# Amandaynzhou/MMT-PSM

Hardware: AMD Instinct MI355X
Metric: imgs/sec (student+teacher step, 1000x1000, AUG_K=2) (higher is better)
Workload: dtype f32

## Files before the change

### include/mmtpsm.h

```cpp
#ifndef MMTPSM_H
#define MMTPSM_H
#include <stdint.h>
#ifdef __cplusplus
extern "C" {
#endif

#define MMT_EINVAL (-22)

int mmt_version(void);

typedef struct {
  const float* feat[4];
  float* grad_feat[4];
  int H[4];
  int W[4];
  float scale[4];
  int num_levels;
  int N;
  int C;
} mmt_pyramid;

int mmt_roi_align_forward(const mmt_pyramid* pyr , const float* rois, const int32_t* levels,
                          int K, int PH, int PW, int sampling_ratio, float* out, void* stream);
int mmt_roi_align_forward_bf16(const mmt_pyramid* pyr , const float* rois, const int32_t* levels,
// ... 103 lines not shown
  const float* res;
  const float* mask;
  const float* mul;
  float* y;
  int N, H, W, Cin, Cout, KH, KW, stride, pad, Ho, Wo;
  int relu, res_mode, out_stride, out_H, out_W;
  float mask_scale;
  const void* w_planes;
  long w_plane_stride;
  const void* x_planes;
  long x_plane_stride;
  void* y_planes;
  long y_plane_stride;
  int io_bf16;
  void* y_amax;
  const void* f16_x_amax;
  const void* f16_dy_amax;
  int y_amax_stats;
  const void* f16_guard_x;
  const void* f16_guard_dy;
  const void* w_src;
  const void* w_src_scale;
  int x_planes_layout;
  void* y_rb;
  long y_rb_stride;
  const float* y_rb_scale;
  void* y_amax_next;
  int x_planes_lag;
  int y_rb_rows;
} mmt_conv_args;

int mmt_conv_forward(const mmt_conv_args* a , void* stream);
int mmt_conv_variant(const mmt_conv_args* a );
int mmt_conv_ksplit(const mmt_conv_args* a );
int mmt_conv_wants_planes(const mmt_conv_args* a );
int mmt_set_conv_precision(int mode);
int mmt_amax(const float* x, long n, const float* rowscale, long inner, int rows, float* amax , void* stream);
int mmt_amax_stats(const float* x, long n, float* slot , void* stream);
int mmt_sum_stats(const float* a, const float* b, const float* c, const float* d, float* y, long n,
                  float* slot , void* stream);
int mmt_stats_combine(const float* const* slots , int n, float* out , void* stream);
int mmt_split_planes_f16(const float* x, void* planes, long plane_stride, long n, float scale, const float* amax ,
                         float* scale_out , float* amax_next ,
                         float* zero_slot , void* stream);
int mmt_pack_weight_f16(const float* w, void* planes, long plane_stride, int Cout, int K, float scale, const float* amax,
                        float* scale_out, void* stream);
int mmt_pack_weight_flipped_f16(const float* w, const float* scale, void* planes, long plane_stride, int Cout, int KH, int KW,
                                int Cin, const float* amax, float* scale_out, void* stream);
int mmt_conv3x3_strip_f16x2(const mmt_conv_args* a , const float* s_x , const float* s_w , void* stream);
int mmt_conv_forward_f16x2(const mmt_conv_args* a , const float* x_amax , const float* s_w , void* stream);
int mmt_get_conv_precision(void);
int mmt_stem_fused(const float* x, int N, int H, int W, const float* w_s2d, const void* w_planes, long w_plane_stride,
                   const float* s_w , const float* scale, const float* shift, const float* x_slot , float* y,
                   float* y_slot , void* stream);
int mmt_c64_conv3_fused(const float* x, int N, int H, int W, const float* w2, const void* w2_planes, long w2_plane_stride,
                        const float* s_w2 , const float* scale2, const float* shift2, const float* x_slot ,
                        const float* w3, const void* w3_planes, long w3_plane_stride, const float* s_w3 , const float* scale3,
                        const float* shift3, const float* res, float* out, float* out_slot ,
                        const float* o2_scale , int o2_scale_is_amax, float* o2_amax_next ,
                        float* out_amax_next , const float* w1, const void* w1_planes, long w1_plane_stride,
                        const float* s_w1 , const float* scale1, const float* shift1, const float* out_scale ,
                        float* o1_next, float* o1_next_slot , void* stream);
int mmt_conv_wgrad_planes_splits(const mmt_conv_args* a );
int mmt_conv_wgrad_planes(const mmt_conv_args* a , const float* dy, const void* x_planes, long x_plane_stride,
                          const void* dy_planes, long dy_plane_stride, const float* s_x, const float* s_dy, const float* rowscale,
                          float* dw, float* dbias, float* workspace, void* stream);
typedef struct {
  void* fn;
  long a[16];
} mmt_call;
int mmt_replay(const mmt_call* calls , int n, int* failed_index );
int mmt_split_planes_f16_rb(const float* x, void* planes, long plane_stride, int rows, int W, int C, const float* amax,
                            float* scale_out, void* stream);
int mmt_conv_writes_rb(const mmt_conv_args* a );
typedef struct mmt_wgrad_job {
  mmt_conv_args a;
  const float* dy; const float* rowscale; float* dw; float* dbias;
  const void* x_planes; long x_plane_stride; const void* dy_planes; long dy_plane_stride; const float* s_x; const float* s_dy;
} mmt_wgrad_job;
int mmt_conv_wgrad_group_workspace(const mmt_wgrad_job* jobs , int n, long* floats_out );
int mmt_conv_wgrad_group(const mmt_wgrad_job* jobs , int n, float* workspace, long workspace_floats, void* stream);
int mmt_sum_stats_rb(const float* a, const float* b, const float* c, const float* d, float* y, int rows, int W, int C, float* slot,
                     void* planes, long plane_stride, const float* scale, float* amax_next, void* stream);
int mmt_rb_scales_update(float* state, int n, void* stream);
int mmt_conv_forward_pg(const mmt_conv_args* a , const float* s_x , const float* s_w , int tile_rows,
                        int ksplit, void* stream);
int mmt_conv_pg_plan(const mmt_conv_args* a , int* tile_rows, int* ksplit);
int mmt_conv_pg_wanted(const mmt_conv_args* a );
typedef struct { long src_off, dst_off; int Cout, K, unit0, pad; } mmt_pack_desc;
long mmt_packed_weight_elems(int Cout, int K);
int mmt_pack_weight(const float* w, void* planes, long plane_stride, int Cout, int K, void* stream);
int mmt_pack_weight_flipped(const float* w, const float* scale, void* planes, long plane_stride, int Cout, int KH, int KW,
                            int Cin, void* stream);
int mmt_split_planes(const float* x, void* planes, long plane_stride, long n, void* stream);
typedef struct { const float* w; const float* scale; void* dst; long plane_stride; int Cout, KH, KW, Cin, unit0, pad; } mmt_flip_desc;
int mmt_pack_weights_flipped(const mmt_flip_desc* descs , const int* unit_desc , int n_units, void* stream);
int mmt_pack_weights(const float* base, void* planes, long plane_stride, const mmt_pack_desc* descs ,
                     const int* unit_desc , int n_units, void* stream);
int mmt_pack_weights_f16(const float* base, void* planes, long plane_stride, const mmt_pack_desc* descs ,
                         const int* unit_desc , int n_units, int n_descs, float* stat , void* stream);
int mmt_pack_weights_flipped_f16(const mmt_flip_desc* descs , const int* unit_desc , int n_units, int n_descs,
                                 float* stat , void* stream);

int mmt_conv_wgrad_splits(const mmt_conv_args* a );
int mmt_conv_wgrad(const mmt_conv_args* a , const float* dy,
                   const float* rowscale , float* dw, float* dbias ,
                   float* workspace , void* stream);
// ... 103 lines not shown
```

### mmt-psm_amd/csrc/conv_stem.hip

```cpp
#include "conv_shared.h"

namespace {

struct StemP {
  const float* x;
  const unsigned short* wpl; long wpl_stride;
  const float* w;
  const float* scale; const float* shift;
  float* y;
  const float* x_slot;
  const float* s_w;
  unsigned* amax_out; int amax_stats;
  int N, H, W, Hc, Wc, Hp, Wp, tiles_y, tiles_x;
};

constexpr int SPH = 19, SPW = 35, SPIX = SPH * SPW;
constexpr int SPL = 672 * 32;
constexpr int SB_OFF = 2 * SPL;
constexpr int STEM_LDS = 128 * 1024;

__device__ __forceinline__ float stem_exact(const StemP& p, int n, int oy, int ox, int co) {
  float acc = 0.f;
  for (int a = 0; a < 4; a++)
    for (int b = 0; b < 4; b++) {
      const int si = oy - 2 + a, sj = ox - 2 + b;
      if ((unsigned)si >= (unsigned)p.Hc || (unsigned)sj >= (unsigned)p.Wc) continue;
      for (int ch = 0; ch < 16; ch++) {
        const int c = ch & 3;
        if (c == 3) continue;
        const float xv = p.x[(((long)n * 3 + c) * p.H + 2 * si + (ch >> 3)) * p.W + 2 * sj + ((ch >> 2) & 1)];
        acc = fmaf(xv, p.w[((co * 4 + a) * 4 + b) * 16 + ch], acc);
      }
    }
  return acc;
}

__global__ __launch_bounds__(512) void stem_fused_kernel(const StemP p) {
  extern __shared__ __attribute__((aligned(16))) float lds[];
  char* const sm = (char*)lds;
  const int tid = threadIdx.x, lane = tid & 63;
  const int wave = __builtin_amdgcn_readfirstlane(tid >> 6);
  int bid = blockIdx.x;
  const int tx = bid % p.tiles_x; bid /= p.tiles_x;
  const int ty = bid % p.tiles_y;
  const int n = bid / p.tiles_y;
  const int py0 = ty * 7, px0 = tx * 15;
  const int oy0 = 2 * py0 - 1, ox0 = 2 * px0 - 1;
  const int sy0 = oy0 - 2, sx0 = ox0 - 2;
  const F16Guard guard = f16_guard_load(p.x_slot);
  const float sx = f16_scale_of(*p.x_slot);

  if (f16_guard_bad(guard)) {
    float amx = 0.f;
    for (int o = tid; o < 7 * 15 * 64; o += 512) {
      const int co = o & 63, q = (o >> 6) % 15, j = (o >> 6) / 15;
      const int py = py0 + j, px = px0 + q;
      if (py >= p.Hp || px >= p.Wp) continue;
      float m = 0.f;
      for (int dy = -1; dy <= 1; dy++)
        for (int dx = -1; dx <= 1; dx++) {
          const int oy = 2 * py + dy, ox = 2 * px + dx;
          if ((unsigned)oy >= (unsigned)p.Hc || (unsigned)ox >= (unsigned)p.Wc) continue;
          m = fmaxf(m, fmaxf(stem_exact(p, n, oy, ox, co) * p.scale[co] + p.shift[co], 0.f));
        }
      p.y[(((long)n * p.Hp + py) * p.Wp + px) * 64 + co] = m;
      amx = fmaxf(amx, m);
    }
    if (p.amax_out && amx > 0.f) atomicMax(p.amax_out, __builtin_bit_cast(unsigned, amx));
    return;
  }

  {
    const __amdgpu_buffer_rsrc_t rs_b = __builtin_amdgcn_make_buffer_rsrc((void*)p.wpl, 0, 0x7ffffff0, 0x00020000);
#pragma unroll
    for (int i = 0; i < 8; i++) {
      const int item = wave + 8 * i, q = item >> 5, rest = item & 31;
      __builtin_amdgcn_raw_ptr_buffer_load_lds(rs_b, (lds_ptr_t)(sm + SB_OFF + item * 1024), 16,
                                               (int)((q * p.wpl_stride + (long)rest * 512 + lane * 8) * 2), 0, 0, 0);
    }
  }
  typedef float f32x2 __attribute__((ext_vector_type(2)));
#pragma unroll
  for (int rnd = 0; rnd < 3; rnd++) {
    const int item = tid + 512 * rnd;
    if (item < 2 * SPIX) {
      const int pix = item >> 1, bh = item & 1;
      const int pr = pix / SPW, pc = pix - pr * SPW;
      const int si = sy0 + pr, sj = sx0 + pc;
      f32x2 v[3];
      const bool ok = (unsigned)si < (unsigned)p.Hc && (unsigned)sj < (unsigned)p.Wc;
#pragma unroll
      for (int c = 0; c < 3; c++)
        v[c] = ok ? *(const f32x2*)(p.x + (((long)n * 3 + c) * p.H + 2 * si + bh) * p.W + 2 * sj) : f32x2{0.f, 0.f};
      uint2 o0[2], o1[2];
      split4h(f32x4{v[0][0], v[1][0], v[2][0], 0.f}, sx, o0);
      split4h(f32x4{v[0][1], v[1][1], v[2][1], 0.f}, sx, o1);
      char* const dst = sm + pix * 32 + ((bh ^ (pix >> 3)) & 1) * 16;
      *(uint4*)dst = uint4{o0[0].x, o0[0].y, o1[0].x, o1[0].y};
      *(uint4*)(dst + SPL) = uint4{o0[1].x, o0[1].y, o1[1].x, o1[1].y};
    }
  }
  asm volatile("s_waitcnt vmcnt(0) lgkmcnt(0)" ::: "memory");
  __syncthreads();

  const int lr = lane & 31, kh2 = lane >> 5;
  const int boff = SB_OFF + lr * 32 + (((kh2 ^ (lr >> 3)) & 1) << 4);
  auto a_addr = [&](int a, int ta, int tb) {
    const int pidx = (2 * wave + a + ta) * SPW + lr + tb;
    return pidx * 32 + (((kh2 ^ (pidx >> 3)) & 1) << 4);
  };
  f32x16 acc[2][2];
#pragma unroll
  for (int a = 0; a < 2; a++)
#pragma unroll
    for (int b = 0; b < 2; b++)
#pragma unroll
      for (int r = 0; r < 16; r++) acc[a][b][r] = 0.f;
  auto fread = [&](int s, f16x8 (&fa)[2][2], f16x8 (&fb)[2][2]) {
    const int ta = s >> 2, tb = s & 3;
#pragma unroll
    for (int a = 0; a < 2; a++) {
      const int ad = a_addr(a, ta, tb);
      fa[0][a] = *(const f16x8*)(sm + ad);
      fa[1][a] = *(const f16x8*)(sm + ad + SPL);
    }
#pragma unroll
    for (int q = 0; q < 2; q++)
#pragma unroll
      for (int b = 0; b < 2; b++) fb[q][b] = *(const f16x8*)(sm + boff + ((q * 16 + s) * 2 + b) * 1024);
  };
  auto mma = [&](const f16x8 (&fa)[2][2], const f16x8 (&fb)[2][2]) {
#pragma unroll
    for (int pr = 0; pr < 3; pr++) {
      const int qa = pr == 1 ? 1 : 0, qb = pr == 0 ? 1 : 0;
#pragma unroll
      for (int a = 0; a < 2; a++)
#pragma unroll
        for (int b = 0; b < 2; b++)
          acc[a][b] = __builtin_amdgcn_mfma_f32_32x32x16_f16(fa[qa][a], fb[qb][b], acc[a][b], 0, 0, 0);
    }
  };
  {
    f16x8 faP[2][2], fbP[2][2], faQ[2][2], fbQ[2][2];
    fread(0, faP, fbP);
#pragma unroll
    for (int s = 0; s < 16; s += 2) {
      fread(s + 1, faQ, fbQ);
      mma(faP, fbP);
      if (s + 2 < 16) fread(s + 2, faP, fbP);
      mma(faQ, fbQ);
    }
  }
  __syncthreads();

  const int col_l = lane & 31, rq = lane >> 5;
  const float inv = 1.f / (sx * *p.s_w);
  float sc[2], sh[2];
#pragma unroll
  for (int b = 0; b < 2; b++) { sc[b] = p.scale[b * 32 + col_l] * inv; sh[b] = p.shift[b * 32 + col_l]; }
  f32x16 m01[2];
#pragma unroll
  for (int b = 0; b < 2; b++)
#pragma unroll
    for (int r = 0; r < 16; r++) {
      const int ox = ox0 + 8 * (r >> 2) + (r & 3) + 4 * rq;
      const bool cok = (unsigned)ox < (unsigned)p.Wc;
      float v[2];
#pragma unroll
      for (int a = 0; a < 2; a++) {
        const int oy = oy0 + 2 * wave + a;
        const float t = fmaxf(acc[a][b][r] * sc[b] + sh[b], 0.f);
        v[a] = (cok && (unsigned)oy < (unsigned)p.Hc) ? t : 0.f;
      }
      acc[0][b][r] = v[0];
      m01[b][r] = fmaxf(v[0], v[1]);
    }
  float* const xr = lds;
  float* const hv = lds + 8 * 32 * 64;
#pragma unroll
  for (int b = 0; b < 2; b++)
#pragma unroll
    for (int r = 0; r < 16; r++)
      xr[(wave * 32 + 8 * (r >> 2) + (r & 3) + 4 * rq) * 64 + b * 32 + col_l] = acc[0][b][r];
  __syncthreads();
  if (wave < 7) {
#pragma unroll
    for (int b = 0; b < 2; b++)
#pragma unroll
      for (int r = 0; r < 16; r++) {
        const int col = 8 * (r >> 2) + (r & 3) + 4 * rq;
        hv[(wave * 32 + col) * 64 + b * 32 + col_l] = fmaxf(m01[b][r], xr[((wave + 1) * 32 + col) * 64 + b * 32 + col_l]);
      }
  }
  __syncthreads();
  float amx = 0.f, asum = 0.f, acnt = 0.f;
  for (int o = tid; o < 7 * 15 * 16; o += 512) {
    const int c4 = o & 15, q = (o >> 4) % 15, j = (o >> 4) / 15;
    const int py = py0 + j, px = px0 + q;
    if (py >= p.Hp || px >= p.Wp) continue;
    const f32x4* const row = (const f32x4*)(hv + (j * 32 + 2 * q) * 64) + c4;
    const f32x4 t0 = row[0], t1 = row[16], t2 = row[32];
    f32x4 m;
#pragma unroll
    for (int e = 0; e < 4; e++) {
      m[e] = fmaxf(fmaxf(t0[e], t1[e]), t2[e]);
      amx = fmaxf(amx, m[e]);
      asum += m[e];
    }
    acnt += 4.f;
    *(f32x4*)(p.y + (((long)n * p.Hp + py) * p.Wp + px) * 64 + c4 * 4) = m;
  }
  if (p.amax_out) {
    __syncthreads();
    float* const red = lds;
    const bool stats = p.amax_stats && (blockIdx.x & 63) == 0;
#pragma unroll
    for (int o = 32; o > 0; o >>= 1) amx = fmaxf(amx, __shfl_xor(amx, o, 64));
    if (stats) {
#pragma unroll
      for (int o = 32; o > 0; o >>= 1) { asum += __shfl_xor(asum, o, 64); acnt += __shfl_xor(acnt, o, 64); }
    }
    if (lane == 0) { red[wave] = amx; red[16 + wave] = asum; red[32 + wave] = acnt; }
    __syncthreads();
    if (tid == 0) {
      float m = red[0], sm_ = red[16], cn = red[32];
      for (int i = 1; i < 8; i++) { m = fmaxf(m, red[i]); sm_ += red[16 + i]; cn += red[32 + i]; }
      const unsigned bits = __builtin_bit_cast(unsigned, m);
      if (m > 0.f && bits > __hip_atomic_load(p.amax_out, __ATOMIC_RELAXED, __HIP_MEMORY_SCOPE_AGENT)) atomicMax(p.amax_out, bits);
      if (stats && cn > 0.f) {
        const int k = (blockIdx.x >> 6) & 15;
        atomicAdd((float*)p.amax_out + 1 + k, sm_);
        atomicAdd((float*)p.amax_out + 17 + k, cn);
      }
    }
  }
}


struct C64Tail {
  const unsigned short* w3pl; long w3pl_stride;
  const float* w3;
  const float* scale; const float* shift;
  const float* res;
  float* out;
  const float* s_w3;
  const float* s_o2; int s_o2_amax;
  unsigned* o2_amax_next;
  unsigned* amax_out;
  unsigned* out_amax_next;
  const unsigned short* w1pl; long w1pl_stride; const float* w1; const float* scale1; const float* shift1; const float* s_w1;
  const float* s_out; float* o1n; unsigned* amax_o1n;
};
constexpr int C64_PW = 18, C64_PIX = 180, C64_SLAB = 192 * 32, C64_PL = 4 * C64_SLAB, C64_BOFF = 2 * C64_PL;
constexpr int C64_RED = 32768;
constexpr int C64_W1B = 32768;

__device__ __forceinline__ void c64_dma16(const void* g, void* l) {
#if defined(__HIP_DEVICE_COMPILE__)
  const unsigned la = __builtin_amdgcn_readfirstlane((unsigned)(unsigned long)(__attribute__((address_space(3))) char*)l);
  asm volatile("s_mov_b32 m0, %1\n\ts_nop 0\n\tglobal_load_lds_dwordx4 %0, off" ::"v"(g), "s"(la) : "m0", "memory");
#endif
}

__device__ __forceinline__ void c64_tail_exact(const ConvP& p, const C64Tail& t, const float* lds, const int img, const int oy0, const int ox0,
                                               const int wave, const int lane, float& amx, float& asum, float& acnt) {
  const float* const o2 = lds + wave * 2048;
  for (int j = 0; j < 4; j++) {
    const int c = lane + 64 * j;
    const float* const wr = t.w3 + c * 64;
    const float sc = t.scale ? t.scale[c] : 1.f, sh = t.shift ? t.shift[c] : 0.f;
    for (int i = 0; i < 32; i++) {
      const int oy = oy0 + 2 * wave + (i >> 4), ox = ox0 + (i & 15);
      if (oy >= p.Ho || ox >= p.Wo) continue;
      float acc = 0.f;
      for (int k = 0; k < 64; k++) acc = fmaf(o2[i * 64 + k], wr[k], acc);
      const long o = ((long)(img * p.Ho + oy) * p.Wo + ox) * 256 + c;
      float v = acc * sc + sh;
      if (t.res) v += t.res[o];
      v = fmaxf(v, 0.f);
      t.out[o] = v;
      amx = fmaxf(amx, v); asum += v; acnt += 1.f;
    }
  }
}

__device__ __forceinline__ float c64_o2_exact(const ConvP& p, float* lds, const int img, const int oy0, const int ox0, const int wave,
                                              const int lane) {
// ... 497 lines not shown
}

template <int FUSE>
static int launch_c64_form(const ConvP& p, const C64Tail& t, hipStream_t s) {
  constexpr int LDS = C64_BOFF + 2 * 16384;
  static bool done = false;
  if (!done) {
    const hipError_t e = hipFuncSetAttribute((const void*)conv3x3_c64_kernel<FUSE>, hipFuncAttributeMaxDynamicSharedMemorySize, LDS);
    if (e != hipSuccess) return (int)e;
    done = true;
  }
  const int tiles = p.N * ((p.Ho + 7) >> 3) * ((p.Wo + 15) >> 4);
  hipLaunchKernelGGL(conv3x3_c64_kernel<FUSE>, dim3(tiles), dim3(256), LDS, s, p, t);
  MMT_LAUNCH_CHECK();
  return 0;
}

int launch_c64(const ConvP& p, hipStream_t s) { return launch_c64_form<0>(p, C64Tail{}, s); }
}

extern "C" int mmt_c64_conv3_fused(const float* x, int N, int H, int W, const float* w2, const void* w2_planes, long w2_plane_stride,
                                   const float* s_w2, const float* scale2, const float* shift2, const float* x_slot, const float* w3,
                                   const void* w3_planes, long w3_plane_stride, const float* s_w3, const float* scale3,
                                   const float* shift3, const float* res, float* out, float* out_slot, const float* o2_scale,
                                   int o2_scale_is_amax, float* o2_amax_next, float* out_amax_next, const float* w1,
                                   const void* w1_planes, long w1_plane_stride, const float* s_w1, const float* scale1,
                                   const float* shift1, const float* out_scale, float* o1_next, float* o1_next_slot, void* stream) {
  if (!x || !w2 || !w2_planes || !s_w2 || !x_slot || !w3 || !w3_planes || !s_w3 || !res || !out || !o2_scale || N <= 0 || H <= 0 || W <= 0 ||
      (((size_t)w2_planes | (size_t)w3_planes | (size_t)x) & 15) || ((w2_plane_stride | w3_plane_stride) & 7) ||
      (((size_t)res | (size_t)out) & 3) || precision() != 3)
    return MMT_EINVAL;
  if (w1_planes && (!w1 || !s_w1 || !out_scale || !o1_next || ((size_t)w1_planes & 15) || (w1_plane_stride & 7) || ((size_t)o1_next & 3) ||
                    (const void*)res == (const void*)out))
    return MMT_EINVAL;
  if ((long)N * H * W * 1024 >= (1L << 31)) return MMT_EINVAL;
  ConvP p = {};
  p.x = x; p.w = w2; p.scale = scale2; p.shift = shift2;
  p.N = N; p.H = p.Ho = H; p.W = p.Wo = W; p.Cin = p.Cout = 64; p.KH = p.KW = 3; p.stride = 1; p.pad = 1;
  p.relu = 1; p.out_stride = 1; p.M = N * H * W; p.K = 576; p.cin32 = p.cin4 = 1;
  p.wpl = (const unsigned short*)w2_planes; p.wpl_stride = w2_plane_stride;
  p.f16_sx = x_slot; p.f16_ax = 1; p.f16_sw = s_w2; p.guard_x = x_slot;
  C64Tail t = {};
  t.w3pl = (const unsigned short*)w3_planes; t.w3pl_stride = w3_plane_stride; t.w3 = w3; t.scale = scale3; t.shift = shift3;
  t.res = res; t.out = out; t.s_w3 = s_w3; t.s_o2 = o2_scale; t.s_o2_amax = o2_scale_is_amax ? 1 : 0;
  t.o2_amax_next = (unsigned*)o2_amax_next; t.amax_out = (unsigned*)out_slot; t.out_amax_next = (unsigned*)out_amax_next;
  if (!w1_planes) return launch_c64_form<1>(p, t, (hipStream_t)stream);
  t.w1pl = (const unsigned short*)w1_planes; t.w1pl_stride = w1_plane_stride; t.w1 = w1; t.scale1 = scale1; t.shift1 = shift1;
  t.s_w1 = s_w1; t.s_out = out_scale; t.o1n = o1_next; t.amax_o1n = (unsigned*)o1_next_slot;
  return launch_c64_form<2>(p, t, (hipStream_t)stream);
}

extern "C" int mmt_stem_fused(const float* x, int N, int H, int W, const float* w_s2d, const void* w_planes, long w_plane_stride,
                              const float* s_w, const float* scale, const float* shift, const float* x_slot, float* y, float* y_slot,
                              void* stream) {
  if (!x || !w_s2d || !w_planes || !s_w || !scale || !shift || !x_slot || !y || N <= 0 || H < 8 || W < 8 || (H & 3) || (W & 3) ||
      ((size_t)w_planes & 15) || (w_plane_stride & 7) || ((size_t)x & 7) || ((size_t)y & 15) || precision() != 3)
    return MMT_EINVAL;
  if ((long)N * 3 * H * W >= (1L << 31)) return MMT_EINVAL;
  StemP p;
  p.x = x; p.wpl = (const unsigned short*)w_planes; p.wpl_stride = w_plane_stride; p.w = w_s2d;
  p.scale = scale; p.shift = shift; p.y = y; p.x_slot = x_slot; p.s_w = s_w;
  p.amax_out = (unsigned*)y_slot; p.amax_stats = y_slot ? 1 : 0;
  p.N = N; p.H = H; p.W = W; p.Hc = H / 2; p.Wc = W / 2; p.Hp = H / 4; p.Wp = W / 4;
  p.tiles_y = mmt_cdiv(p.Hp, 7); p.tiles_x = mmt_cdiv(p.Wp, 15);
  static bool done = false;
  if (!done) {
    const hipError_t e = hipFuncSetAttribute((const void*)stem_fused_kernel, hipFuncAttributeMaxDynamicSharedMemorySize, STEM_LDS);
    if (e != hipSuccess) return (int)e;
    done = true;
  }
  hipLaunchKernelGGL(stem_fused_kernel, dim3(N * p.tiles_y * p.tiles_x), dim3(512), STEM_LDS, (hipStream_t)stream, p);
  MMT_LAUNCH_CHECK();
  return 0;
}
```

### mmt-psm_amd/maskrcnn_benchmark/_hip.py

```python
import ctypes
import weakref
import os
import threading as _threading

import torch

_HERE = os.path.dirname(os.path.abspath(__file__))
LIB_PATH = os.path.join(os.path.dirname(_HERE), "libmmtpsm.so")

c_void_p, c_int, c_float, c_double, c_int64 = ctypes.c_void_p, ctypes.c_int, ctypes.c_float, ctypes.c_double, ctypes.c_int64


class Pyramid(ctypes.Structure):
    _fields_ = [("feat", c_void_p * 4), ("grad_feat", c_void_p * 4), ("H", c_int * 4), ("W", c_int * 4),
                ("scale", c_float * 4), ("num_levels", c_int), ("N", c_int), ("C", c_int)]


class RoiMaps(ctypes.Structure):
    _fields_ = [("feat", c_void_p * 4), ("grad_feat", c_void_p * 4), ("H", c_int * 4), ("W", c_int * 4), ("C", c_int * 4),
                ("c_off", c_int * 4), ("scale", c_float * 4), ("num_maps", c_int), ("N", c_int), ("out_C", c_int)]


class ConvArgs(ctypes.Structure):
    _fields_ = [("x", c_void_p), ("w", c_void_p), ("scale", c_void_p), ("shift", c_void_p), ("res", c_void_p),
# ... 86 lines not shown
                       c_void_p, c_void_p],
    "mmt_split_planes": [c_void_p, c_void_p, ctypes.c_long, ctypes.c_long, c_void_p],
    "mmt_conv_wants_planes": [ctypes.POINTER(ConvArgs)],
    "mmt_pack_weights": [c_void_p, c_void_p, ctypes.c_long, c_void_p, c_void_p, c_int, c_void_p],
    "mmt_pack_weights_flipped": [c_void_p, c_void_p, c_int, c_void_p],
    "mmt_pack_weights_f16": [c_void_p, c_void_p, ctypes.c_long, c_void_p, c_void_p, c_int, c_int, c_void_p, c_void_p],
    "mmt_pack_weights_flipped_f16": [c_void_p, c_void_p, c_int, c_int, c_void_p, c_void_p],
    "mmt_pack_weight_flipped": [c_void_p, c_void_p, c_void_p, ctypes.c_long, c_int, c_int, c_int, c_int, c_void_p],
    "mmt_conv_wgrad_splits": [ctypes.POINTER(ConvArgs)],
    "mmt_conv_wgrad": [ctypes.POINTER(ConvArgs), c_void_p, c_void_p, c_void_p, c_void_p, c_void_p, c_void_p],
    "mmt_colsum": [c_void_p, c_int, c_int, c_void_p, c_void_p],
    "mmt_weight_flip_transpose": [c_void_p, c_void_p, c_void_p, c_int, c_int, c_int, c_int, c_void_p],
    "mmt_maxpool3x3s2": [c_void_p, c_void_p, c_int, c_int, c_int, c_int, c_int, c_int, c_void_p],
    "mmt_amax": [c_void_p, ctypes.c_long, c_void_p, ctypes.c_long, c_int, c_void_p, c_void_p],
    "mmt_amax_stats": [c_void_p, ctypes.c_long, c_void_p, c_void_p],
    "mmt_det_postprocess": [c_void_p, c_void_p, c_void_p, c_void_p, c_int, c_int, c_float, c_float, c_int, c_void_p,
                            c_void_p, c_void_p, c_void_p, c_void_p, c_void_p],
    "mmt_position_embedding": [c_void_p, c_int, c_int, c_int, c_void_p, c_void_p, c_void_p],
    "mmt_sample_fg_bg_wide": [c_void_p, c_int, c_void_p, c_void_p, c_int, c_int, c_int, c_int, c_void_p, c_void_p, c_void_p, c_void_p,
                              c_void_p],
    "mmt_rpn_loss": [c_void_p, c_void_p, c_void_p, c_void_p, c_void_p, c_void_p, ctypes.c_long, c_float, c_void_p, c_void_p, c_void_p,
                     c_void_p, c_void_p],
    "mmt_box_loss": [c_void_p, c_void_p, c_void_p, c_void_p, c_int, c_int, c_void_p, c_void_p, c_void_p, c_void_p],
    "mmt_box_loss_rows": [c_void_p, c_void_p, c_void_p, c_void_p, c_int, c_int, c_void_p, c_void_p, c_void_p, c_void_p, c_void_p],
    "mmt_relation_attention_fwd": [c_void_p, c_void_p, c_void_p, c_void_p, c_void_p, c_int, c_int, c_int, c_int, c_int, c_int, c_float,
                                   c_void_p, c_void_p, c_void_p],
    "mmt_relation_attention_bwd": [c_void_p, c_void_p, c_void_p, c_void_p, c_void_p, c_void_p, c_int, c_int, c_int, c_int, c_int, c_float,
                                   c_void_p, c_void_p, c_void_p, c_void_p, c_void_p, c_void_p],
    "mmt_ciam_fwd": [c_void_p, c_void_p, c_int, c_int, c_int, c_int, c_void_p, c_void_p, c_void_p, c_void_p, c_void_p],
    "mmt_ciam_bwd": [c_void_p, c_void_p, c_int, c_int, c_int, c_int, c_void_p, c_void_p, c_void_p, c_void_p, c_void_p, c_void_p,
                     c_void_p, c_void_p, c_void_p],
    "mmt_stats_combine": [c_void_p, c_int, c_void_p, c_void_p],
    "mmt_sum_stats": [c_void_p, c_void_p, c_void_p, c_void_p, c_void_p, ctypes.c_long, c_void_p, c_void_p],
    "mmt_split_planes_f16": [c_void_p, c_void_p, ctypes.c_long, ctypes.c_long, c_float, c_void_p, c_void_p, c_void_p, c_void_p, c_void_p],
    "mmt_split_planes_f16_rb": [c_void_p, c_void_p, ctypes.c_long, c_int, c_int, c_int, c_void_p, c_void_p, c_void_p],
    "mmt_replay": [c_void_p, c_int, c_void_p],
    "mmt_conv_writes_rb": [ctypes.POINTER(ConvArgs)],
    "mmt_conv_wgrad_group_workspace": [c_void_p, c_int, ctypes.POINTER(ctypes.c_long)],
    "mmt_conv_wgrad_group": [c_void_p, c_int, c_void_p, ctypes.c_long, c_void_p],
    "mmt_sum_stats_rb": [c_void_p, c_void_p, c_void_p, c_void_p, c_void_p, c_int, c_int, c_int, c_void_p, c_void_p, ctypes.c_long, c_void_p,
                         c_void_p, c_void_p],
    "mmt_rb_scales_update": [c_void_p, c_int, c_void_p],
    "mmt_conv_wgrad_planes_splits": [ctypes.POINTER(ConvArgs)],
    "mmt_conv_wgrad_planes": [ctypes.POINTER(ConvArgs), c_void_p, c_void_p, ctypes.c_long, c_void_p, ctypes.c_long, c_void_p, c_void_p,
                              c_void_p, c_void_p, c_void_p, c_void_p, c_void_p],
    "mmt_pack_weight_f16": [c_void_p, c_void_p, ctypes.c_long, c_int, c_int, c_float, c_void_p, c_void_p, c_void_p],
    "mmt_pack_weight_flipped_f16": [c_void_p, c_void_p, c_void_p, ctypes.c_long, c_int, c_int, c_int, c_int, c_void_p, c_void_p, c_void_p],
    "mmt_conv3x3_strip_f16x2": [ctypes.POINTER(ConvArgs), c_void_p, c_void_p, c_void_p],
    "mmt_conv_forward_f16x2": [ctypes.POINTER(ConvArgs), c_void_p, c_void_p, c_void_p],
    "mmt_conv_forward_pg": [ctypes.POINTER(ConvArgs), c_void_p, c_void_p, c_int, c_int, c_void_p],
    "mmt_conv_pg_plan": [ctypes.POINTER(ConvArgs), c_void_p, c_void_p],
    "mmt_conv_pg_wanted": [ctypes.POINTER(ConvArgs)],
    "mmt_stem_fused": [c_void_p, c_int, c_int, c_int, c_void_p, c_void_p, ctypes.c_long, c_void_p, c_void_p, c_void_p, c_void_p, c_void_p,
                       c_void_p, c_void_p],
    "mmt_c64_conv3_fused": [c_void_p, c_int, c_int, c_int, c_void_p, c_void_p, ctypes.c_long, c_void_p, c_void_p, c_void_p, c_void_p, c_void_p,
                            c_void_p, ctypes.c_long, c_void_p, c_void_p, c_void_p, c_void_p, c_void_p, c_void_p, c_void_p, c_int, c_void_p,
                            c_void_p, c_void_p, c_void_p, ctypes.c_long, c_void_p, c_void_p, c_void_p, c_void_p, c_void_p, c_void_p,
                            c_void_p],
    "mmt_maxpool3x3s2_bf16": [c_void_p, c_void_p, c_int, c_int, c_int, c_int, c_int, c_int, c_void_p],
    "mmt_gconv3x3_forward": [c_void_p, c_void_p, c_void_p, c_void_p, c_void_p, c_int, c_int, c_int, c_int, c_int, c_int, c_int, c_void_p],
    "mmt_gconv3x3_dgrad": [c_void_p, c_void_p, c_void_p, c_void_p, c_void_p, c_void_p, c_int, c_int, c_int, c_int, c_int, c_int, c_void_p],
    "mmt_gconv3x3_wgrad": [c_void_p, c_void_p, c_void_p, c_void_p, c_int, c_int, c_int, c_int, c_int, c_int, c_void_p],
    "mmt_maxpool3x3s2_backward": [c_void_p, c_void_p, c_void_p, c_int, c_int, c_int, c_int, c_void_p],
    "mmt_stem_wgrad": [c_void_p, c_void_p, c_void_p, c_void_p, c_int, c_int, c_int, c_void_p],
    "mmt_mask_bce": [c_void_p, c_void_p, c_void_p, c_int, c_int, c_int, c_float, c_void_p, c_void_p, c_void_p],
    "mmt_mgd_level_forward": [c_void_p, ctypes.POINTER(MgdTeachers), c_void_p, c_int, c_int, c_int, c_int, c_void_p, c_void_p],
    "mmt_mgd_level_backward": [c_void_p, ctypes.POINTER(MgdTeachers), c_void_p, c_int, c_int, c_int, c_int, c_void_p, c_void_p, c_void_p],
    "mmt_mgd_views_forward": [ctypes.POINTER(MgdStudents), ctypes.POINTER(MgdTeachers), c_void_p, c_int, c_int, c_int, c_int, c_void_p,
                              c_void_p],
    "mmt_mgd_views_backward": [ctypes.POINTER(MgdStudents), ctypes.POINTER(MgdTeachers), c_void_p, c_int, c_int, c_int, c_int, c_void_p,
                               c_void_p, c_void_p],
    "mmt_mask_pool": [c_void_p, c_int, c_int, c_int, c_int, c_int, c_void_p, c_void_p],
    "mmt_psm_rows": [c_void_p, c_int, c_void_p, c_int, c_int, c_void_p, c_float, c_int, c_int, c_void_p, c_void_p, c_void_p],
    "mmt_psm_variance": [c_void_p, c_int, c_int, c_int, c_int, c_void_p, c_void_p],
    "mmt_ema_update": [c_void_p, c_void_p, c_int64, c_double, c_void_p],
    "mmt_sgd_momentum": [c_void_p, c_void_p, c_void_p, c_int64, c_float, c_float, c_float, c_int, c_void_p],
    "mmt_grad_guard": [c_void_p, c_int64, c_void_p, c_void_p, c_float, c_void_p],
    "mmt_sgd_momentum_guarded": [c_void_p, c_void_p, c_void_p, c_int64, c_float, c_float, c_float, c_int, c_void_p, c_void_p],
    "mmt_paste_masks": [c_void_p, c_void_p, c_void_p, c_void_p, c_int, c_int, c_int, c_int, c_int, c_float, c_void_p, c_void_p],
    "mmt_paste_mask_stack": [c_void_p, c_void_p, c_int, c_int, c_int, c_int, c_float, c_void_p, c_void_p],
    "mmt_polygon_targets": [c_void_p, c_void_p, c_void_p, c_void_p, c_int, c_int, c_void_p, c_void_p, c_void_p],
    "mmt_mask_pack": [c_void_p, c_int, c_int, c_int, c_void_p, c_void_p, c_void_p],
    "mmt_paste_mask_words": [c_void_p, c_void_p, c_int, c_int, c_int, c_int, c_float, c_void_p, c_void_p, c_void_p],
    "mmt_mask_expand": [c_void_p, c_void_p, c_int, c_int, c_int, c_void_p, c_void_p, c_void_p],
    "mmt_mask_transition_counts": [c_void_p, c_int, c_int, c_int, c_void_p, c_void_p],
    "mmt_mask_transition_positions": [c_void_p, c_int, c_int, c_int, c_void_p, c_void_p, c_void_p],
    "mmt_mask_pair_intersections": [c_void_p, c_void_p, c_int, c_void_p, c_void_p, c_int, c_int, c_int, c_void_p, c_void_p],
    "mmt_set_deterministic": [c_int],
    "mmt_get_deterministic": [],
    "mmt_roi_align_backward_ordered": [ctypes.POINTER(Pyramid), c_void_p, c_void_p, c_int, c_int, c_int, c_int, c_void_p, c_int, c_void_p],
    "mmt_colsum_ordered": [c_void_p, c_int, c_int, c_void_p, c_void_p, c_void_p],
    "mmt_mask_bce_ordered": [c_void_p, c_void_p, c_void_p, c_int, c_int, c_int, c_float, c_void_p, c_void_p, c_void_p, c_void_p],
    "mmt_mgd_level_forward_ordered": [c_void_p, ctypes.POINTER(MgdTeachers), c_void_p, c_int, c_int, c_int, c_int, c_void_p, c_void_p, c_void_p],
    "mmt_mgd_views_forward_ordered": [ctypes.POINTER(MgdStudents), ctypes.POINTER(MgdTeachers), c_void_p, c_int, c_int, c_int, c_int, c_void_p,
                                      c_void_p, c_void_p],
    "mmt_box_loss_ordered": [c_void_p, c_void_p, c_void_p, c_void_p, c_int, c_int, c_void_p, c_void_p, c_void_p, c_void_p, c_void_p, c_void_p],
    "mmt_ciam_bwd_ordered": [c_void_p, c_void_p, c_int, c_int, c_int, c_int, c_void_p, c_void_p, c_void_p, c_void_p, c_void_p, c_void_p,
                             c_void_p, c_void_p, c_void_p, c_void_p],
}

_lib = None
PROFILE = None
PROFILE_ALL = False
_BF16_STORAGE = os.environ.get("MMT_BF16_STORAGE", "0") != "0"


F16X2_DEFAULT = os.environ.get("MMT_F16X2", "1") != "0"
# ... 1486 lines not shown
        a.y_amax, a.y_amax_stats = amax_slot.ptr, 1
    if mul is not None:
        mul = nhwc(mul)
        a.mul = mul.data_ptr()
    ebytes = _epilogue_bytes(y, res, res_mode, mask, mul) if PROFILE is not None else None
    if kind != K_LIB:
        if fast_ok and not io:
            _plan_record(x, w, f16_src, stride, pad, relu, res, res_mode, mask, a, kind, Cout, Ho, Wo)
        if amax_slot is None or mul is not None:
            rb_site = None
        return _conv_f16(a, kind, x, src, y, amax_slot, rb_site, 0, 0, None, ebytes)
    var = lib().mmt_conv_variant(ctypes.byref(a)) if ebytes is not None else 0
    rec = ebytes is not None and (var in (1, 4) or PROFILE_ALL)
    pre = None
    if auto_split:
        p0 = _ev() if rec else None
        split_planes(x, x_planes)
        if rec:
            pre = (p0, _ev())
    e0 = _ev() if rec else None
    if planes_owner is not None:
        planes_owner.ensure_bf16()
    _check(lib().mmt_conv_forward(ctypes.byref(a), _stream()), "mmt_conv_forward")
    if rec:
        _profiled(a, e0, "fwd%d" % var, lib().mmt_conv_ksplit(ctypes.byref(a)), pre, ebytes)
    if y_planes is not None:
        y._mmt_planes = (y_planes, y._version)
    if amax_slot is not None:
        y._mmt_amax = (amax_slot, y._version)
    return y


def conv_forward_pg(x, w, scale=None, shift=None, stride=1, pad=0, relu=False, res=None, mask=None, mask_scale=1.0, w_shape=None,
                    f16_src=None, tile_rows=0, ksplit=0, xp=None):
    x = nhwc(x)
    N, Cin, H, W = x.shape
    src = (nhwc(w), False, None) if w is not None else (nhwc(f16_src[0]), True, f16_src[1])
    Cout, KH, KW = _weight_dims(Cin, src[0].shape if w is not None else w_shape)
    Ho, Wo = _conv_out_hw(H, W, KH, KW, stride, pad)
    a = _conv_shape(ConvArgs(), N, H, W, Cin, Cout, KH, KW, stride, pad, Ho, Wo)
    a.x = x.data_ptr()
    y = empty_nhwc(N, Cout, Ho, Wo, x.device)
    a.y = y.data_ptr()
    a.scale, a.shift, a.relu = _p(scale), _p(shift), 1 if relu else 0
    if res is not None:
        a.res, a.res_mode = nhwc(res).data_ptr(), 1
    if mask is not None:
        a.mask, a.mask_scale = nhwc(mask).data_ptr(), float(mask_scale)
    slot = _amax_slot(x.device)
    a.y_amax, a.y_amax_stats = slot.ptr, 1
    return _conv_f16(a, K_PG, x, src, y, slot, None, int(tile_rows), int(ksplit), xp, None, False)


def stem_fused(x, w_s2d, scale, shift):
    _dev(x)
    N, C, Hh, W = x.shape
    if C != 3 or not x.is_contiguous() or x.dtype != torch.float32 or (Hh & 3) or (W & 3) or tuple(w_s2d.shape) != (64, 16, 4, 4):
        raise RuntimeError("stem_fused: (N, 3, H, W) fp32 NCHW with H, W % 4 == 0 and the 64 x 16 x 4 x 4 space-to-depth filter")
    w = nhwc(w_s2d)
    am = _amax_of(x)
    if type(am[0]) is not _Slot:
        raise RuntimeError("stem_fused: the input needs a full statistics slot")
    wp16, sw = f16_weight_planes(w)
    y = empty_nhwc(N, 64, Hh // 4, W // 4, x.device)
    slot = _amax_slot(x.device)
    _check(lib().mmt_stem_fused(x.data_ptr(), N, Hh, W, w.data_ptr(), wp16.data_ptr(), wp16.stride(0), sw.data_ptr(), _p(scale), _p(shift),
                                am[0].ptr, y.data_ptr(), slot.ptr, _stream()), "mmt_stem_fused")
    y._mmt_amax = (slot, y._version)
    return y


C64_FUSE = os.environ.get("MMT_C64_FUSE", "1") != "0"


def o2_site(w3):
    return ("o2", w3.data_ptr())


def c64_fuse_enabled():
    return bool(C64_FUSE and F16X2 and RB_EPI and PROFILE is None and os.environ.get("MMT_C64") != "0" and get_conv_precision() == 3)


def out_site(w1_next):
    return ("out1", w1_next.data_ptr())


def c64_conv3_fused(x, w2, scale2, shift2, w3, scale3, shift3, res, o2_amax=None, nxt=None, out_amax=None):
    if not c64_fuse_enabled():
        return None
    N, C, Hh, W = x.shape
    if (C != 64 or tuple(w2.shape) != (64, 64, 3, 3) or tuple(w3.shape) != (256, 64, 1, 1) or tuple(res.shape) != (N, 256, Hh, W)
            or x.dtype != torch.float32 or res.dtype != torch.float32 or N * Hh * W >= (1 << 21) or N * Hh * W == 0):
        return None
    if nxt is not None and tuple(nxt[0].shape) != (64, 256, 1, 1):
        return None
    site = o2_site(w3)
    x, res, w2, w3 = nhwc(x), nhwc(res), nhwc(w2), nhwc(w3)
    if not _site_ok((w2.data_ptr(), False), x, count=False):
        return None
    pend = None
    if o2_amax is None:
        t, i = _rb_site(site, x.device)
        if t is None or i not in t.ready:
            return None
        t.produced.add(i)
        sc, pend = t.base + 8 * i, t.base + 8 * i + 4
    else:
        sc = o2_amax.data_ptr()
    am = _amax_of(x)
    if type(am[0]) is not _Slot:
        return None
    wp2, sw2 = f16_weight_planes(w2)
    wp3, sw3 = f16_weight_planes(w3)
    out = empty_nhwc(N, 256, Hh, W, x.device)
    slot = _amax_slot(x.device)
    nx = [None] * 10
    nx[3] = 0
    o1n = nslot = None
    if nxt is not None:
        w1 = nhwc(nxt[0])
# ... 873 lines not shown
```

Before: 130.4.

## Make stem conv kernel persistent with prefetch of next tile's input

The fused stem conv+BN+ReLU+maxpool kernel becomes a persistent kernel launched with one block per CU (or a caller-given count) that loops over tiles. The weight planes are loaded into LDS once per block, and the global loads of the next tile's input are issued into registers before the current tile's MFMA work, so load latency overlaps compute. LDS use is cut from 128 KiB to about 128 KiB total with the stage reused, and the per-tile amax reduction moves to per-wave atomics at the end. The cost is higher register pressure from the prefetch buffers, extra barriers per tile, and a change to which tiles contribute to the sampled sum/count statistics.

Measured after the change: 129.8. Within noise of the previous version (-0.5%).

```diff
diff --git a/include/mmtpsm.h b/include/mmtpsm.h
--- a/include/mmtpsm.h
+++ b/include/mmtpsm.h
@@ -179,7 +179,7 @@
 int mmt_get_conv_precision(void);
 int mmt_stem_fused(const float* x, int N, int H, int W, const float* w_s2d, const void* w_planes, long w_plane_stride,
                    const float* s_w , const float* scale, const float* shift, const float* x_slot , float* y,
-                   float* y_slot , void* stream);
+                   float* y_slot , int blocks, void* stream);
 int mmt_c64_conv3_fused(const float* x, int N, int H, int W, const float* w2, const void* w2_planes, long w2_plane_stride,
                         const float* s_w2 , const float* scale2, const float* shift2, const float* x_slot ,
                         const float* w3, const void* w3_planes, long w3_plane_stride, const float* s_w3 , const float* scale3,
diff --git a/mmt-psm_amd/csrc/conv_stem.hip b/mmt-psm_amd/csrc/conv_stem.hip
--- a/mmt-psm_amd/csrc/conv_stem.hip
+++ b/mmt-psm_amd/csrc/conv_stem.hip
@@ -16,8 +16,10 @@
 
 constexpr int SPH = 19, SPW = 35, SPIX = SPH * SPW;
 constexpr int SPL = 672 * 32;
-constexpr int SB_OFF = 2 * SPL;
-constexpr int STEM_LDS = 128 * 1024;
+constexpr int STEM_STAGE = 8 * 32 * 64 * 4;
+constexpr int SB_OFF = STEM_STAGE;
+constexpr int STEM_LDS = SB_OFF + 64 * 1024;
+static_assert(2 * SPL <= STEM_STAGE, "the patch planes lie inside the stage's LDS");
 
 __device__ __forceinline__ float stem_exact(const StemP& p, int n, int oy, int ox, int co) {
   float acc = 0.f;
@@ -39,37 +41,78 @@
   extern __shared__ __attribute__((aligned(16))) float lds[];
   char* const sm = (char*)lds;
   const int tid = threadIdx.x, lane = tid & 63;
-  const int wave = __builtin_amdgcn_readfirstlane(tid >> 6);
-  int bid = blockIdx.x;
-  const int tx = bid % p.tiles_x; bid /= p.tiles_x;
-  const int ty = bid % p.tiles_y;
-  const int n = bid / p.tiles_y;
-  const int py0 = ty * 7, px0 = tx * 15;
-  const int oy0 = 2 * py0 - 1, ox0 = 2 * px0 - 1;
-  const int sy0 = oy0 - 2, sx0 = ox0 - 2;
+  int wave = __builtin_amdgcn_readfirstlane(tid >> 6);
+  const int tiles = p.N * p.tiles_y * p.tiles_x, stride = gridDim.x;
   const F16Guard guard = f16_guard_load(p.x_slot);
   const float sx = f16_scale_of(*p.x_slot);
 
   if (f16_guard_bad(guard)) {
     float amx = 0.f;
-    for (int o = tid; o < 7 * 15 * 64; o += 512) {
-      const int co = o & 63, q = (o >> 6) % 15, j = (o >> 6) / 15;
-      const int py = py0 + j, px = px0 + q;
-      if (py >= p.Hp || px >= p.Wp) continue;
-      float m = 0.f;
-      for (int dy = -1; dy <= 1; dy++)
-        for (int dx = -1; dx <= 1; dx++) {
-          const int oy = 2 * py + dy, ox = 2 * px + dx;
-          if ((unsigned)oy >= (unsigned)p.Hc || (unsigned)ox >= (unsigned)p.Wc) continue;
-          m = fmaxf(m, fmaxf(stem_exact(p, n, oy, ox, co) * p.scale[co] + p.shift[co], 0.f));
-        }
-      p.y[(((long)n * p.Hp + py) * p.Wp + px) * 64 + co] = m;
-      amx = fmaxf(amx, m);
+    for (int tile = blockIdx.x; tile < tiles; tile += stride) {
+      const int n = tile / (p.tiles_y * p.tiles_x), py0 = tile / p.tiles_x % p.tiles_y * 7, px0 = tile % p.tiles_x * 15;
+      for (int o = tid; o < 7 * 15 * 64; o += 512) {
+        const int co = o & 63, q = (o >> 6) % 15, j = (o >> 6) / 15;
+        const int py = py0 + j, px = px0 + q;
+        if (py >= p.Hp || px >= p.Wp) continue;
+        float m = 0.f;
+        for (int dy = -1; dy <= 1; dy++)
+          for (int dx = -1; dx <= 1; dx++) {
+            const int oy = 2 * py + dy, ox = 2 * px + dx;
+            if ((unsigned)oy >= (unsigned)p.Hc || (unsigned)ox >= (unsigned)p.Wc) continue;
+            m = fmaxf(m, fmaxf(stem_exact(p, n, oy, ox, co) * p.scale[co] + p.shift[co], 0.f));
+          }
+        p.y[(((long)n * p.Hp + py) * p.Wp + px) * 64 + co] = m;
+        amx = fmaxf(amx, m);
+      }
     }
     if (p.amax_out && amx > 0.f) atomicMax(p.amax_out, __builtin_bit_cast(unsigned, amx));
     return;
   }
 
+  typedef float f32x2 __attribute__((ext_vector_type(2)));
+  f32x2 gv[3][3];
+  int tidv = tid, lr = lane & 31, kh2 = lane >> 5;
+  int g_pr[3], g_pc[3];
+  long g_off[3];
+#pragma unroll
+  for (int rnd = 0; rnd < 3; rnd++) {
+    const int item = tid + 512 * rnd;
+    const int pix = item >> 1, bh = item & 1;
+    const int pr = pix / SPW, pc = pix - pr * SPW;
+    g_pr[rnd] = item < 2 * SPIX ? pr : 1 << 29;
+    g_pc[rnd] = pc;
+    g_off[rnd] = (long)(2 * pr + bh) * p.W + 2 * pc;
+  }
+  auto request = [&](const int tile) {
+    const int n = tile / (p.tiles_y * p.tiles_x);
+    const int sy0 = tile / p.tiles_x % p.tiles_y * 14 - 3, sx0 = tile % p.tiles_x * 30 - 3;
+    const long base = ((long)n * 3 * p.H + 2 * sy0) * p.W + 2 * sx0, plane = (long)p.H * p.W;
+#pragma unroll
+    for (int rnd = 0; rnd < 3; rnd++) {
+      const bool ok = (unsigned)(sy0 + g_pr[rnd]) < (unsigned)p.Hc && (unsigned)(sx0 + g_pc[rnd]) < (unsigned)p.Wc;
+#pragma unroll
+      for (int c = 0; c < 3; c++)
+        gv[rnd][c] = ok ? *(const f32x2*)(p.x + (base + c * plane) + g_off[rnd]) : f32x2{0.f, 0.f};
+    }
+    asm volatile("" ::: "memory");
+  };
+  auto split = [&]() {
+#pragma unroll
+    for (int rnd = 0; rnd < 3; rnd++) {
+      const int item = tidv + 512 * rnd;
+      if (item < 2 * SPIX) {
+        const int pix = item >> 1, bh = item & 1;
+        uint2 o0[2], o1[2];
+        split4h(f32x4{gv[rnd][0][0], gv[rnd][1][0], gv[rnd][2][0], 0.f}, sx, o0);
+        split4h(f32x4{gv[rnd][0][1], gv[rnd][1][1], gv[rnd][2][1], 0.f}, sx, o1);
+        char* const dst = sm + pix * 32 + ((bh ^ (pix >> 3)) & 1) * 16;
+        *(uint4*)dst = uint4{o0[0].x, o0[0].y, o1[0].x, o1[0].y};
+        *(uint4*)(dst + SPL) = uint4{o0[1].x, o0[1].y, o1[1].x, o1[1].y};
+      }
+    }
+  };
+  int tile = blockIdx.x;
+  if (tile < tiles) request(tile);
   {
     const __amdgpu_buffer_rsrc_t rs_b = __builtin_amdgcn_make_buffer_rsrc((void*)p.wpl, 0, 0x7ffffff0, 0x00020000);
 #pragma unroll
@@ -79,43 +122,21 @@
                                                (int)((q * p.wpl_stride + (long)rest * 512 + lane * 8) * 2), 0, 0, 0);
     }
   }
-  typedef float f32x2 __attribute__((ext_vector_type(2)));
-#pragma unroll
-  for (int rnd = 0; rnd < 3; rnd++) {
-    const int item = tid + 512 * rnd;
-    if (item < 2 * SPIX) {
-      const int pix = item >> 1, bh = item & 1;
-      const int pr = pix / SPW, pc = pix - pr * SPW;
-      const int si = sy0 + pr, sj = sx0 + pc;
-      f32x2 v[3];
-      const bool ok = (unsigned)si < (unsigned)p.Hc && (unsigned)sj < (unsigned)p.Wc;
-#pragma unroll
-      for (int c = 0; c < 3; c++)
-        v[c] = ok ? *(const f32x2*)(p.x + (((long)n * 3 + c) * p.H + 2 * si + bh) * p.W + 2 * sj) : f32x2{0.f, 0.f};
-      uint2 o0[2], o1[2];
-      split4h(f32x4{v[0][0], v[1][0], v[2][0], 0.f}, sx, o0);
-      split4h(f32x4{v[0][1], v[1][1], v[2][1], 0.f}, sx, o1);
-      char* const dst = sm + pix * 32 + ((bh ^ (pix >> 3)) & 1) * 16;
-      *(uint4*)dst = uint4{o0[0].x, o0[0].y, o1[0].x, o1[0].y};
-      *(uint4*)(dst + SPL) = uint4{o0[1].x, o0[1].y, o1[1].x, o1[1].y};
-    }
-  }
+  if (tile < tiles) split();
   asm volatile("s_waitcnt vmcnt(0) lgkmcnt(0)" ::: "memory");
-  __syncthreads();
-
-  const int lr = lane & 31, kh2 = lane >> 5;
+
+  float sc[2], sh[2];
+  {
+    const float inv = 1.f / (sx * *p.s_w);
+#pragma unroll
+    for (int b = 0; b < 2; b++) { sc[b] = p.scale[b * 32 + (lane & 31)] * inv; sh[b] = p.shift[b * 32 + (lane & 31)]; }
+  }
   const int boff = SB_OFF + lr * 32 + (((kh2 ^ (lr >> 3)) & 1) << 4);
   auto a_addr = [&](int a, int ta, int tb) {
     const int pidx = (2 * wave + a + ta) * SPW + lr + tb;
     return pidx * 32 + (((kh2 ^ (pidx >> 3)) & 1) << 4);
   };
   f32x16 acc[2][2];
-#pragma unroll
-  for (int a = 0; a < 2; a++)
-#pragma unroll
-    for (int b = 0; b < 2; b++)
-#pragma unroll
-      for (int r = 0; r < 16; r++) acc[a][b][r] = 0.f;
   auto fread = [&](int s, f16x8 (&fa)[2][2], f16x8 (&fb)[2][2]) {
     const int ta = s >> 2, tb = s & 3;
 #pragma unroll
@@ -140,99 +161,120 @@
           acc[a][b] = __builtin_amdgcn_mfma_f32_32x32x16_f16(fa[qa][a], fb[qb][b], acc[a][b], 0, 0, 0);
     }
   };
-  {
-    f16x8 faP[2][2], fbP[2][2], faQ[2][2], fbQ[2][2];
-    fread(0, faP, fbP);
-#pragma unroll
-    for (int s = 0; s < 16; s += 2) {
-      fread(s + 1, faQ, fbQ);
-      mma(faP, fbP);
-      if (s + 2 < 16) fread(s + 2, faP, fbP);
-      mma(faQ, fbQ);
-    }
-  }
-  __syncthreads();
-
-  const int col_l = lane & 31, rq = lane >> 5;
-  const float inv = 1.f / (sx * *p.s_w);
-  float sc[2], sh[2];
-#pragma unroll
-  for (int b = 0; b < 2; b++) { sc[b] = p.scale[b * 32 + col_l] * inv; sh[b] = p.shift[b * 32 + col_l]; }
-  f32x16 m01[2];
-#pragma unroll
-  for (int b = 0; b < 2; b++)
-#pragma unroll
-    for (int r = 0; r < 16; r++) {
-      const int ox = ox0 + 8 * (r >> 2) + (r & 3) + 4 * rq;
-      const bool cok = (unsigned)ox < (unsigned)p.Wc;
-      float v[2];
-#pragma unroll
-      for (int a = 0; a < 2; a++) {
-        const int oy = oy0 + 2 * wave + a;
-        const float t = fmaxf(acc[a][b][r] * sc[b] + sh[b], 0.f);
-        v[a] = (cok && (unsigned)oy < (unsigned)p.Hc) ? t : 0.f;
-      }
-      acc[0][b][r] = v[0];
-      m01[b][r] = fmaxf(v[0], v[1]);
-    }
   float* const xr = lds;
-  float* const hv = lds + 8 * 32 * 64;
-#pragma unroll
-  for (int b = 0; b < 2; b++)
-#pragma unroll
-    for (int r = 0; r < 16; r++)
-      xr[(wave * 32 + 8 * (r >> 2) + (r & 3) + 4 * rq) * 64 + b * 32 + col_l] = acc[0][b][r];
-  __syncthreads();
-  if (wave < 7) {
+  float* const hv = lds + 32 * 64;
+  float amx = 0.f;
+
+  for (; tile < tiles; tile += stride) {
+    const int n = tile / (p.tiles_y * p.tiles_x), py0 = tile / p.tiles_x % p.tiles_y * 7, px0 = tile % p.tiles_x * 15;
+    const int oy0 = 2 * py0 - 1, ox0 = 2 * px0 - 1;
+    const bool more = tile + stride < tiles;
+    {
+      int ln = lane;
+      asm volatile("" : "+v"(ln), "+s"(wave));
+      tidv = wave * 64 + ln; lr = ln & 31; kh2 = ln >> 5;
+    }
+    const int col_l = lr, rq = kh2;
+    __syncthreads();
+    if (more) request(tile + stride);
+#pragma unroll
+    for (int a = 0; a < 2; a++)
+#pragma unroll
+      for (int b = 0; b < 2; b++)
+#pragma unroll
+        for (int r = 0; r < 16; r++) acc[a][b][r] = 0.f;
+    {
+      f16x8 faP[2][2], fbP[2][2], faQ[2][2], fbQ[2][2];
+      fread(0, faP, fbP);
+#pragma unroll
+      for (int s = 0; s < 16; s += 2) {
+        fread(s + 1, faQ, fbQ);
+        mma(faP, fbP);
+        if (s + 2 < 16) fread(s + 2, faP, fbP);
+        mma(faQ, fbQ);
+      }
+    }
+    __syncthreads();
+
+    f32x16 m01[2];
 #pragma unroll
     for (int b = 0; b < 2; b++)
 #pragma unroll
       for (int r = 0; r < 16; r++) {
-        const int col = 8 * (r >> 2) + (r & 3) + 4 * rq;
-        hv[(wave * 32 + col) * 64 + b * 32 + col_l] = fmaxf(m01[b][r], xr[((wave + 1) * 32 + col) * 64 + b * 32 + col_l]);
-      }
-  }
-  __syncthreads();
-  float amx = 0.f, asum = 0.f, acnt = 0.f;
-  for (int o = tid; o < 7 * 15 * 16; o += 512) {
-    const int c4 = o & 15, q = (o >> 4) % 15, j = (o >> 4) / 15;
-    const int py = py0 + j, px = px0 + q;
-    if (py >= p.Hp || px >= p.Wp) continue;
-    const f32x4* const row = (const f32x4*)(hv + (j * 32 + 2 * q) * 64) + c4;
-    const f32x4 t0 = row[0], t1 = row[16], t2 = row[32];
-    f32x4 m;
-#pragma unroll
-    for (int e = 0; e < 4; e++) {
-      m[e] = fmaxf(fmaxf(t0[e], t1[e]), t2[e]);
-      amx = fmaxf(amx, m[e]);
-      asum += m[e];
-    }
-    acnt += 4.f;
-    *(f32x4*)(p.y + (((long)n * p.Hp + py) * p.Wp + px) * 64 + c4 * 4) = m;
+        const int ox = ox0 + 8 * (r >> 2) + (r & 3) + 4 * rq;
+        const bool cok = (unsigned)ox < (unsigned)p.Wc;
+        float v[2];
+#pragma unroll
+        for (int a = 0; a < 2; a++) {
+          const int oy = oy0 + 2 * wave + a;
+          const float t = fmaxf(acc[a][b][r] * sc[b] + sh[b], 0.f);
+          v[a] = (cok && (unsigned)oy < (unsigned)p.Hc) ? t : 0.f;
+        }
+        acc[0][b][r] = v[0];
+        m01[b][r] = fmaxf(v[0], v[1]);
+      }
+#pragma unroll
+    for (int b = 0; b < 2; b++)
+#pragma unroll
+      for (int r = 0; r < 16; r++)
+        xr[(wave * 32 + 8 * (r >> 2) + (r & 3) + 4 * rq) * 64 + b * 32 + col_l] = acc[0][b][r];
+    __syncthreads();
+    if (wave < 7) {
+#pragma unroll
+      for (int b = 0; b < 2; b++)
+#pragma unroll
+        for (int r = 0; r < 16; r++) {
+          const int col = 8 * (r >> 2) + (r & 3) + 4 * rq;
+          float* const e = xr + ((wave + 1) * 32 + col) * 64 + b * 32 + col_l;
+          *e = fmaxf(m01[b][r], *e);
+        }
+    }
+    __syncthreads();
+    f32x4 pm[4];
+    float asum = 0.f, acnt = 0.f;
+#pragma unroll
+    for (int i = 0; i < 4; i++) {
+      const int o = tidv + 512 * i;
+      const int c4 = o & 15, q = (o >> 4) % 15, j = (o >> 4) / 15;
+      pm[i] = f32x4{0.f, 0.f, 0.f, 0.f};
+      if (o < 7 * 15 * 16 && py0 + j < p.Hp && px0 + q < p.Wp) {
+        const f32x4* const row = (const f32x4*)(hv + (j * 32 + 2 * q) * 64) + c4;
+        const f32x4 t0 = row[0], t1 = row[16], t2 = row[32];
+#pragma unroll
+        for (int e = 0; e < 4; e++) {
+          pm[i][e] = fmaxf(fmaxf(t0[e], t1[e]), t2[e]);
+          amx = fmaxf(amx, pm[i][e]);
+          asum += pm[i][e];
+        }
+        acnt += 4.f;
+      }
+    }
+    if (more) {
+      __syncthreads();
+      split();
+    }
+#pragma unroll
+    for (int i = 0; i < 4; i++) {
+      const int o = tidv + 512 * i;
+      const int c4 = o & 15, q = (o >> 4) % 15, j = (o >> 4) / 15;
+      if (o < 7 * 15 * 16 && py0 + j < p.Hp && px0 + q < p.Wp)
+        *(f32x4*)(p.y + (((long)n * p.Hp + py0 + j) * p.Wp + px0 + q) * 64 + c4 * 4) = pm[i];
+    }
+    if (p.amax_stats && (tile & 63) == 0) {
+#pragma unroll
+      for (int o = 32; o > 0; o >>= 1) { asum += __shfl_xor(asum, o, 64); acnt += __shfl_xor(acnt, o, 64); }
+      if (lane == 0 && acnt > 0.f) {
+        const int k = (tile >> 6) & 15;
+        atomicAdd((float*)p.amax_out + 1 + k, asum);
+        atomicAdd((float*)p.amax_out + 17 + k, acnt);
+      }
+    }
   }
   if (p.amax_out) {
-    __syncthreads();
-    float* const red = lds;
-    const bool stats = p.amax_stats && (blockIdx.x & 63) == 0;
 #pragma unroll
     for (int o = 32; o > 0; o >>= 1) amx = fmaxf(amx, __shfl_xor(amx, o, 64));
-    if (stats) {
-#pragma unroll
-      for (int o = 32; o > 0; o >>= 1) { asum += __shfl_xor(asum, o, 64); acnt += __shfl_xor(acnt, o, 64); }
-    }
-    if (lane == 0) { red[wave] = amx; red[16 + wave] = asum; red[32 + wave] = acnt; }
-    __syncthreads();
-    if (tid == 0) {
-      float m = red[0], sm_ = red[16], cn = red[32];
-      for (int i = 1; i < 8; i++) { m = fmaxf(m, red[i]); sm_ += red[16 + i]; cn += red[32 + i]; }
-      const unsigned bits = __builtin_bit_cast(unsigned, m);
-      if (m > 0.f && bits > __hip_atomic_load(p.amax_out, __ATOMIC_RELAXED, __HIP_MEMORY_SCOPE_AGENT)) atomicMax(p.amax_out, bits);
-      if (stats && cn > 0.f) {
-        const int k = (blockIdx.x >> 6) & 15;
-        atomicAdd((float*)p.amax_out + 1 + k, sm_);
-        atomicAdd((float*)p.amax_out + 17 + k, cn);
-      }
-    }
+    const unsigned bits = __builtin_bit_cast(unsigned, amx);
+    if (lane == 0 && amx > 0.f && bits > __hip_atomic_load(p.amax_out, __ATOMIC_RELAXED, __HIP_MEMORY_SCOPE_AGENT)) atomicMax(p.amax_out, bits);
   }
 }
 
@@ -836,8 +878,8 @@
 
 extern "C" int mmt_stem_fused(const float* x, int N, int H, int W, const float* w_s2d, const void* w_planes, long w_plane_stride,
                               const float* s_w, const float* scale, const float* shift, const float* x_slot, float* y, float* y_slot,
-                              void* stream) {
-  if (!x || !w_s2d || !w_planes || !s_w || !scale || !shift || !x_slot || !y || N <= 0 || H < 8 || W < 8 || (H & 3) || (W & 3) ||
+                              int blocks, void* stream) {
+  if (!x || !w_s2d || !w_planes || !s_w || !scale || !shift || !x_slot || !y || N <= 0 || H < 8 || W < 8 || (H & 3) || (W & 3) || blocks < 0 ||
       ((size_t)w_planes & 15) || (w_plane_stride & 7) || ((size_t)x & 7) || ((size_t)y & 15) || precision() != 3)
     return MMT_EINVAL;
   if ((long)N * 3 * H * W >= (1L << 31)) return MMT_EINVAL;
@@ -853,7 +895,15 @@
     if (e != hipSuccess) return (int)e;
     done = true;
   }
-  hipLaunchKernelGGL(stem_fused_kernel, dim3(N * p.tiles_y * p.tiles_x), dim3(512), STEM_LDS, (hipStream_t)stream, p);
+  const int tiles = N * p.tiles_y * p.tiles_x;
+  if (!blocks) {
+    static int cus[64];
+    int dev = 0;
+    if (hipGetDevice(&dev) != hipSuccess || dev < 0 || dev >= 64) return MMT_EINVAL;
+    if (!cus[dev] && hipDeviceGetAttribute(&cus[dev], hipDeviceAttributeMultiprocessorCount, dev) != hipSuccess) return MMT_EINVAL;
+    blocks = cus[dev] > 0 ? cus[dev] : 256;
+  }
+  hipLaunchKernelGGL(stem_fused_kernel, dim3(blocks < tiles ? blocks : tiles), dim3(512), STEM_LDS, (hipStream_t)stream, p);
   MMT_LAUNCH_CHECK();
   return 0;
 }
diff --git a/mmt-psm_amd/maskrcnn_benchmark/_hip.py b/mmt-psm_amd/maskrcnn_benchmark/_hip.py
--- a/mmt-psm_amd/maskrcnn_benchmark/_hip.py
+++ b/mmt-psm_amd/maskrcnn_benchmark/_hip.py
@@ -162,7 +162,7 @@
     "mmt_conv_pg_plan": [ctypes.POINTER(ConvArgs), c_void_p, c_void_p],
     "mmt_conv_pg_wanted": [ctypes.POINTER(ConvArgs)],
     "mmt_stem_fused": [c_void_p, c_int, c_int, c_int, c_void_p, c_void_p, ctypes.c_long, c_void_p, c_void_p, c_void_p, c_void_p, c_void_p,
-                       c_void_p, c_void_p],
+                       c_void_p, c_int, c_void_p],
     "mmt_c64_conv3_fused": [c_void_p, c_int, c_int, c_int, c_void_p, c_void_p, ctypes.c_long, c_void_p, c_void_p, c_void_p, c_void_p, c_void_p,
                             c_void_p, ctypes.c_long, c_void_p, c_void_p, c_void_p, c_void_p, c_void_p, c_void_p, c_void_p, c_int, c_void_p,
                             c_void_p, c_void_p, c_void_p, ctypes.c_long, c_void_p, c_void_p, c_void_p, c_void_p, c_void_p, c_void_p,
@@ -1755,7 +1755,7 @@
     return _conv_f16(a, K_PG, x, src, y, slot, None, int(tile_rows), int(ksplit), xp, None, False)
 
 
-def stem_fused(x, w_s2d, scale, shift):
+def stem_fused(x, w_s2d, scale, shift, blocks=0):
     _dev(x)
     N, C, Hh, W = x.shape
     if C != 3 or not x.is_contiguous() or x.dtype != torch.float32 or (Hh & 3) or (W & 3) or tuple(w_s2d.shape) != (64, 16, 4, 4):
@@ -1768,7 +1768,7 @@
     y = empty_nhwc(N, 64, Hh // 4, W // 4, x.device)
     slot = _amax_slot(x.device)
     _check(lib().mmt_stem_fused(x.data_ptr(), N, Hh, W, w.data_ptr(), wp16.data_ptr(), wp16.stride(0), sw.data_ptr(), _p(scale), _p(shift),
-                                am[0].ptr, y.data_ptr(), slot.ptr, _stream()), "mmt_stem_fused")
+                                am[0].ptr, y.data_ptr(), slot.ptr, int(blocks), _stream()), "mmt_stem_fused")
     y._mmt_amax = (slot, y._version)
     return y
 
```
